# SADPR/1D-Burgers-Equation-ROMs

Hardware: AMD Instinct MI355X
Metric: batched Newton-steps/sec over mu-sweep (sample-Newton-steps/s, FOM N=1024) (higher is better)
Workload: dtype f64

## Files before the change

### 1d-burgers-equation-roms_amd/csrc/fom.hip

```cpp
#include <hip/hip_runtime.h>
#include <stdint.h>
#include <type_traits>

#include "../../include/burgers_hip.h"
#include "abi_common.hpp"
#include "fom_device.hpp"
#include "fom_wide.hpp"

namespace bg {
thread_local int tls_last_hip_error = 0;
}

namespace {

using namespace bg;

struct FomArgs {
    const double* x;
    const double* u0;
    const double* mu1;
    const double* mu2;
    double* hist;
    int32_t* iters;
    int32_t* flags;
    double dt, E, tol2;
    int N, B, nsteps, max_it, supg;
    double* errs;
};

constexpr int WAVES_PER_WG = 4;

template <int R>
__device__ __forceinline__ void load_rows(const double* __restrict__ src, int N, int row0, bool full,
                                          double (&u)[R])
{
#pragma unroll
    for (int j = 0; j < R; ++j) u[j] = (full || row0 + j < N) ? src[row0 + j] : 0.0;
}

template <int R>
__device__ __forceinline__ void store_rows(double* __restrict__ dst, int N, int row0, bool full,
                                           const double (&u)[R])
{
#pragma unroll
    for (int j = 0; j < R; ++j)
        if (full || row0 + j < N) dst[row0 + j] = u[j];
}

template <int R, bool FULL, bool UNI = true, bool TRACE = false>
__global__ __launch_bounds__(64 * WAVES_PER_WG, 1) void fom_fused_kernel(FomArgs a)
{
    const int lane = lane_id();
    const int s = blockIdx.x * WAVES_PER_WG + (int)(threadIdx.x >> 6);
    if (s >= a.B) return;
    const int N = a.N;
    const int row0 = lane * R;
    const double h = (a.x[N - 1] - a.x[0]) / (double)(N - 1);
    const MeshConst c = make_mesh_const(h, a.dt, a.E, a.supg);
    const double mu1 = a.mu1[s], mu2 = a.mu2[s];

    double hfs[R], fdt[R], u[R], g[R];
    ElemGeom<UNI ? 0 : R> gm;
    if constexpr (UNI) {
        forcing_setup<R>(a.x, N, row0, mu2, c.h, a.dt, hfs, fdt);
    } else {
        geom_setup<R>(a.x, N, row0, a.dt, a.E, gm);
        forcing_setup_general<R>(a.x, N, row0, mu2, a.dt, hfs, fdt);
    }

    double* hist = a.hist + (size_t)s * (size_t)(a.nsteps + 1) * (size_t)N;
    load_rows<R>(a.u0 + (size_t)s * N, N, row0, FULL, u);
    store_rows<R>(hist, N, row0, FULL, u);

    int flags = 0;
    for (int step = 0; step < a.nsteps; ++step) {
        if constexpr (UNI) mass_rhs<R, FULL>(c, N, row0, u, fdt, g);
        else mass_rhs_general<R>(gm, N, row0, u, fdt, g);
        int k = 0;
        bool more;
        do {
            double lo[R], di[R], up[R], rhs[R];
            if constexpr (UNI) assemble<R, FULL>(c, N, row0, mu1, u, g, hfs, lo, di, up, rhs);
            else assemble_general<R>(gm, a.dt, c.kap, N, row0, mu1, u, g, hfs, lo, di, up, rhs);
            tridiag_solve<R>(lo, di, up, rhs);
            double nd = 0.0, nu = 0.0;
#pragma unroll
            for (int j = 0; j < R; ++j) {
                u[j] += rhs[j];
                nd = __builtin_fma(rhs[j], rhs[j], nd);
                nu = __builtin_fma(u[j], u[j], nu);
            }
            wave_sum2(nd, nu, nd, nu);
            if constexpr (TRACE) {
                if (lane == 0) a.errs[((size_t)s * a.nsteps + step) * a.max_it + k] = sqrt(nd) / sqrt(nu);
            }
            ++k;
            more = (nd > a.tol2 * nu) && (k < a.max_it);
            if (!(nd - nd == 0.0) || !(nu - nu == 0.0)) flags |= BG_FLAG_NONFINITE;
        } while (more);
        if (k >= a.max_it) flags |= BG_FLAG_HIT_CAP;
        store_rows<R>(hist + (size_t)(step + 1) * N, N, row0, FULL, u);
        if (lane == 0) a.iters[(size_t)s * a.nsteps + step] = k;
    }
    if (lane == 0) a.flags[s] = flags;
}

struct AsmArgs {
    const double *x, *uk, *un, *mu1, *mu2;
    double *lo, *di, *up, *rhs;
    double dt, E;
    int N, B, supg;
};

template <int R, bool FULL, bool UNI = true>
__global__ __launch_bounds__(64 * WAVES_PER_WG, 1) void fom_assemble_kernel(AsmArgs a)
{
    const int lane = lane_id();
    const int s = blockIdx.x * WAVES_PER_WG + (int)(threadIdx.x >> 6);
    if (s >= a.B) return;
    const int N = a.N, row0 = lane * R;
    const double h = (a.x[N - 1] - a.x[0]) / (double)(N - 1);
    const MeshConst c = make_mesh_const(h, a.dt, a.E, a.supg);
    double hfs[R], fdt[R], u[R], un[R], g[R], lo[R], di[R], up[R], rhs[R];
    load_rows<R>(a.un + (size_t)s * N, N, row0, FULL, un);
    load_rows<R>(a.uk + (size_t)s * N, N, row0, FULL, u);
    if constexpr (UNI) {
        forcing_setup<R>(a.x, N, row0, a.mu2[s], c.h, a.dt, hfs, fdt);
        mass_rhs<R, FULL>(c, N, row0, un, fdt, g);
        assemble<R, FULL>(c, N, row0, a.mu1[s], u, g, hfs, lo, di, up, rhs);
    } else {
        ElemGeom<R> gm;
        geom_setup<R>(a.x, N, row0, a.dt, a.E, gm);
        forcing_setup_general<R>(a.x, N, row0, a.mu2[s], a.dt, hfs, fdt);
        mass_rhs_general<R>(gm, N, row0, un, fdt, g);
        assemble_general<R>(gm, a.dt, c.kap, N, row0, a.mu1[s], u, g, hfs, lo, di, up, rhs);
    }
    store_rows<R>(a.lo + (size_t)s * N, N, row0, FULL, lo);
    store_rows<R>(a.di + (size_t)s * N, N, row0, FULL, di);
    store_rows<R>(a.up + (size_t)s * N, N, row0, FULL, up);
    store_rows<R>(a.rhs + (size_t)s * N, N, row0, FULL, rhs);
}

struct SolveArgs {
    const double *lo, *di, *up, *rhs;
    double* sol;
    int N, B;
};

template <int R>
__global__ __launch_bounds__(64 * WAVES_PER_WG, 1) void tridiag_solve_kernel(SolveArgs a)
{
    const int lane = lane_id();
    const int s = blockIdx.x * WAVES_PER_WG + (int)(threadIdx.x >> 6);
    if (s >= a.B) return;
    const int N = a.N, row0 = lane * R;
    double lo[R], di[R], up[R], rhs[R];
    const size_t off = (size_t)s * N;
#pragma unroll
    for (int j = 0; j < R; ++j) {
        const bool in = row0 + j < N;
        lo[j] = in ? a.lo[off + row0 + j] : 0.0;
        di[j] = in ? a.di[off + row0 + j] : 1.0;
        up[j] = in ? a.up[off + row0 + j] : 0.0;
        rhs[j] = in ? a.rhs[off + row0 + j] : 0.0;
    }
    tridiag_solve<R>(lo, di, up, rhs);
    store_rows<R>(a.sol + off, N, row0, false, rhs);
}

template <int R, bool UNI>
__global__ __launch_bounds__(WIDE_THREADS, 1) void fom_wide_kernel(FomArgs a)
{
    constexpr bool PARK = UNI && R >= 32;
    __shared__ WideLds lds;
    __shared__ WidePark<PARK ? R : 1> park;
    const int g = threadIdx.x, s = blockIdx.x;
    const int N = a.N, row0 = g * R;
    wide_init(lds, g);
    const double h = (a.x[N - 1] - a.x[0]) / (double)(N - 1);
    const MeshConst c = make_mesh_const(h, a.dt, a.E, a.supg);
    const double mu1 = a.mu1[s], mu2 = a.mu2[s];
    double hfs[PARK ? 1 : R], fdt[R], u[R], gv[PARK ? 1 : R];
    ElemGeom<UNI ? 0 : R> gm;
    if constexpr (PARK) {
        double hf[R];
        forcing_setup<R>(a.x, N, row0, mu2, c.h, a.dt, hf, fdt);
#pragma unroll
        for (int j = 0; j < R; ++j) park.hfs[j][g] = hf[j];
    } else if constexpr (UNI) {
        forcing_setup<R>(a.x, N, row0, mu2, c.h, a.dt, hfs, fdt);
    } else {
        geom_setup<R>(a.x, N, row0, a.dt, a.E, gm);
        forcing_setup_general<R>(a.x, N, row0, mu2, a.dt, hfs, fdt);
    }
    double* hist = a.hist + (size_t)s * (size_t)(a.nsteps + 1) * (size_t)N;
    load_rows<R>(a.u0 + (size_t)s * N, N, row0, false, u);
    store_rows<R>(hist, N, row0, false, u);
    int flags = 0;
    for (int step = 0; step < a.nsteps; ++step) {
        if constexpr (PARK) wide_mass_rhs_uni_parked<R>(lds, park, g, c, N, u, fdt);
        else if constexpr (UNI) wide_mass_rhs_uni<R>(lds, g, c, N, u, fdt, gv);
        else wide_mass_rhs<R>(lds, g, gm, N, u, fdt, gv);
        int k = 0;
        bool more;
        do {
            double lo[R], di[R], up[R], rhs[R];
            if constexpr (PARK) wide_assemble_uni_parked<R>(lds, park, g, c, N, mu1, u, lo, di, up, rhs);
            else if constexpr (UNI) wide_assemble_uni<R>(lds, g, c, N, mu1, u, gv, hfs, lo, di, up, rhs);
            else wide_assemble<R>(lds, g, gm, a.dt, c.kap, N, mu1, u, gv, hfs, lo, di, up, rhs);
            wide_tridiag_solve<R>(lds, g, lo, di, up, rhs);
            double nd = 0.0, nu = 0.0;
#pragma unroll
            for (int j = 0; j < R; ++j) {
                u[j] += rhs[j];
                nd = __builtin_fma(rhs[j], rhs[j], nd);
                nu = __builtin_fma(u[j], u[j], nu);
            }
            wide_sum2(lds, g, nd, nu, nd, nu);
            ++k;
            more = (nd > a.tol2 * nu) && (k < a.max_it);
            if (!(nd - nd == 0.0) || !(nu - nu == 0.0)) flags |= BG_FLAG_NONFINITE;
        } while (more);
        if (k >= a.max_it) flags |= BG_FLAG_HIT_CAP;
        store_rows<R>(hist + (size_t)(step + 1) * N, N, row0, false, u);
        if (g == 0) a.iters[(size_t)s * a.nsteps + step] = k;
    }
    if (g == 0) a.flags[s] = flags;
}

template <int R, bool UNI>
__global__ __launch_bounds__(WIDE_THREADS, 1) void fom_assemble_wide_kernel(AsmArgs a)
{
    __shared__ WideLds lds;
    const int g = threadIdx.x, s = blockIdx.x;
    const int N = a.N, row0 = g * R;
    wide_init(lds, g);
    const double h = (a.x[N - 1] - a.x[0]) / (double)(N - 1);
    const MeshConst c = make_mesh_const(h, a.dt, a.E, a.supg);
    double hfs[R], fdt[R], u[R], un[R], gv[R], lo[R], di[R], up[R], rhs[R];
    load_rows<R>(a.un + (size_t)s * N, N, row0, false, un);
    load_rows<R>(a.uk + (size_t)s * N, N, row0, false, u);
    if constexpr (UNI) {
        forcing_setup<R>(a.x, N, row0, a.mu2[s], c.h, a.dt, hfs, fdt);
        wide_mass_rhs_uni<R>(lds, g, c, N, un, fdt, gv);
        wide_assemble_uni<R>(lds, g, c, N, a.mu1[s], u, gv, hfs, lo, di, up, rhs);
    } else {
        ElemGeom<R> gm;
        geom_setup<R>(a.x, N, row0, a.dt, a.E, gm);
        forcing_setup_general<R>(a.x, N, row0, a.mu2[s], a.dt, hfs, fdt);
        wide_mass_rhs<R>(lds, g, gm, N, un, fdt, gv);
        wide_assemble<R>(lds, g, gm, a.dt, c.kap, N, a.mu1[s], u, gv, hfs, lo, di, up, rhs);
    }
    store_rows<R>(a.lo + (size_t)s * N, N, row0, false, lo);
    store_rows<R>(a.di + (size_t)s * N, N, row0, false, di);
    store_rows<R>(a.up + (size_t)s * N, N, row0, false, up);
    store_rows<R>(a.rhs + (size_t)s * N, N, row0, false, rhs);
}

template <int R>
__global__ __launch_bounds__(WIDE_THREADS, 1) void tridiag_solve_wide_kernel(SolveArgs a)
{
    __shared__ WideLds lds;
    const int g = threadIdx.x, s = blockIdx.x;
    const int N = a.N, row0 = g * R;
    wide_init(lds, g);
    double lo[R], di[R], up[R], rhs[R];
    const size_t off = (size_t)s * N;
#pragma unroll
    for (int j = 0; j < R; ++j) {
        const bool in = row0 + j < N;
        lo[j] = in ? a.lo[off + row0 + j] : 0.0;
        di[j] = in ? a.di[off + row0 + j] : 1.0;
        up[j] = in ? a.up[off + row0 + j] : 0.0;
        rhs[j] = in ? a.rhs[off + row0 + j] : 0.0;
    }
    wide_tridiag_solve<R>(lds, g, lo, di, up, rhs);
    store_rows<R>(a.sol + off, N, row0, false, rhs);
}

__global__ __launch_bounds__(256) void transpose_kernel(const double* __restrict__ in,
                                                        double* __restrict__ out, int nb, int rows, int cols)
{
    __shared__ double tile[32][33];
    const int c0 = blockIdx.x * 32, r0 = blockIdx.y * 32;
    const int tx = threadIdx.x & 31, ty = threadIdx.x >> 5;
    for (int b = blockIdx.z; b < nb; b += gridDim.z) {
        const size_t base = (size_t)b * rows * cols;
#pragma unroll
        for (int k = 0; k < 32; k += 8) {
            int r = r0 + ty + k, cc = c0 + tx;
            if (r < rows && cc < cols) tile[ty + k][tx] = in[base + (size_t)r * cols + cc];
        }
        __syncthreads();
#pragma unroll
        for (int k = 0; k < 32; k += 8) {
            int cc = c0 + ty + k, r = r0 + tx;
            if (r < rows && cc < cols) out[base + (size_t)cc * rows + r] = tile[tx][ty + k];
        }
        __syncthreads();
    }
}

constexpr int kRowsPerLane[] = {1, 2, 3, 4, 5, 6, 8, 9, 10, 12, 16, 24};

int rows_per_lane(int N)
{
    for (int r : kRowsPerLane)
        if (N <= 64 * r) return r;
    return 0;
}

constexpr int kWaveMaxN = 64 * 24, kWideMaxN = WIDE_THREADS * 32;

template <typename F>
int dispatch_wide(int N, F&& f)
{
    if (N <= WIDE_THREADS * 2) return f(std::integral_constant<int, 2>{});
    if (N <= WIDE_THREADS * 4) return f(std::integral_constant<int, 4>{});
    if (N <= WIDE_THREADS * 8) return f(std::integral_constant<int, 8>{});
    if (N <= WIDE_THREADS * 12) return f(std::integral_constant<int, 12>{});
    if (N <= WIDE_THREADS * 16) return f(std::integral_constant<int, 16>{});
    if (N <= WIDE_THREADS * 24) return f(std::integral_constant<int, 24>{});
    if (N <= WIDE_THREADS * 32) return f(std::integral_constant<int, 32>{});
    return BG_ERR_UNSUPPORTED_N;
}

template <typename F>
int dispatch_r(int N, F&& f)
{
    switch (rows_per_lane(N)) {
        case 1: return f(std::integral_constant<int, 1>{});
        case 2: return f(std::integral_constant<int, 2>{});
        case 3: return f(std::integral_constant<int, 3>{});
        case 4: return f(std::integral_constant<int, 4>{});
        case 5: return f(std::integral_constant<int, 5>{});
        case 6: return f(std::integral_constant<int, 6>{});
        case 8: return f(std::integral_constant<int, 8>{});
        case 9: return f(std::integral_constant<int, 9>{});
        case 10: return f(std::integral_constant<int, 10>{});
        case 12: return f(std::integral_constant<int, 12>{});
        case 16: return f(std::integral_constant<int, 16>{});
        case 24: return f(std::integral_constant<int, 24>{});
        default: return BG_ERR_UNSUPPORTED_N;
    }
}

}

extern "C" {

int bg_abi_version(void) { return BG_ABI_VERSION; }

int bg_last_hip_error(void) { return bg::tls_last_hip_error; }

int bg_fom_max_n(void) { return kWideMaxN; }

const char* bg_strerror(int code)
{
    switch (code) {
        case BG_OK: return "ok";
        case BG_ERR_BAD_ARG: return "bad argument";
        case BG_ERR_UNSUPPORTED_N: return "N not supported by the fused kernels (2 <= N <= 8192)";
        case BG_ERR_NONUNIFORM: return "mesh is not uniform";
        case BG_ERR_LAUNCH: return "kernel launch failed (see bg_last_hip_error)";
        case BG_ERR_UNSUPPORTED_R: return "reduced dimension not supported";
        case BG_ERR_PROJECTION: return "unknown projection";
        case BG_ERR_WORKSPACE: return "workspace too small";
        default: return "unknown error";
    }
}

int bg_fom_run(int N, int B, int nsteps, const double* x, const double* u0, const double* mu1,
               const double* mu2, double dt, double E, double tol, int max_it, int supg, double* hist,
               int32_t* iters, int32_t* flags, void* stream)
{
    if (N < 2 || B < 0 || nsteps < 0 || max_it < 1 || !(dt > 0.0)) return BG_ERR_BAD_ARG;
    if (B == 0) return BG_OK;
    if (!x || !u0 || !mu1 || !mu2 || !hist || !flags || (nsteps > 0 && !iters)) return BG_ERR_BAD_ARG;
    FomArgs a;
    a.x = x; a.u0 = u0; a.mu1 = mu1; a.mu2 = mu2; a.hist = hist; a.iters = iters; a.flags = flags; a.errs = nullptr;
    a.dt = dt; a.E = E; a.tol2 = tol * tol;
    a.N = N; a.B = B; a.nsteps = nsteps; a.max_it = max_it; a.supg = supg & BG_OPT_SUPG;
    const bool nonuniform = (supg & BG_OPT_NONUNIFORM) != 0;
    const dim3 grid((B + WAVES_PER_WG - 1) / WAVES_PER_WG), block(64 * WAVES_PER_WG);
    hipStream_t st = (hipStream_t)stream;
    const bool both = N <= kWaveMaxN && N > 64 && !nonuniform;
    const bool wide = N > kWaveMaxN || (both && (supg & BG_OPT_FOM_WIDE) && !(supg & BG_OPT_FOM_WAVE));
    if (wide)
        return dispatch_wide(N, [&](auto rc) {
            constexpr int R = decltype(rc)::value;
            if constexpr (R >= 8) {
                if (nonuniform) {
                    hipLaunchKernelGGL((fom_wide_kernel<R, false>), dim3(B), dim3(WIDE_THREADS), 0, st, a);
                    return check_launch();
                }
            }
            hipLaunchKernelGGL((fom_wide_kernel<R, true>), dim3(B), dim3(WIDE_THREADS), 0, st, a);
            return check_launch();
        });
    return dispatch_r(N, [&](auto rc) {
        constexpr int R = decltype(rc)::value;
        if (nonuniform)
            hipLaunchKernelGGL((fom_fused_kernel<R, false, false>), grid, block, 0, st, a);
        else if (N == 64 * R)
            hipLaunchKernelGGL((fom_fused_kernel<R, true>), grid, block, 0, st, a);
        else
            hipLaunchKernelGGL((fom_fused_kernel<R, false>), grid, block, 0, st, a);
        return check_launch();
    });
}

int bg_fom_run_traced(int N, int B, int nsteps, const double* x, const double* u0, const double* mu1, const double* mu2,
                      double dt, double E, double tol, int max_it, int supg, double* hist, int32_t* iters, int32_t* flags,
                      double* errs, void* stream)
{
    if (N < 2 || B < 0 || nsteps < 0 || max_it < 1 || !(dt > 0.0)) return BG_ERR_BAD_ARG;
    if (N > kWaveMaxN) return BG_ERR_UNSUPPORTED_N;
    if (B == 0) return BG_OK;
    if (!x || !u0 || !mu1 || !mu2 || !hist || !flags || !errs || (nsteps > 0 && !iters)) return BG_ERR_BAD_ARG;
    FomArgs a;
    a.x = x; a.u0 = u0; a.mu1 = mu1; a.mu2 = mu2; a.hist = hist; a.iters = iters; a.flags = flags; a.errs = errs;
    a.dt = dt; a.E = E; a.tol2 = tol * tol;
    a.N = N; a.B = B; a.nsteps = nsteps; a.max_it = max_it; a.supg = supg & BG_OPT_SUPG;
    const bool nonuniform = (supg & BG_OPT_NONUNIFORM) != 0;
    const dim3 grid((B + WAVES_PER_WG - 1) / WAVES_PER_WG), block(64 * WAVES_PER_WG);
    hipStream_t st = (hipStream_t)stream;
    return dispatch_r(N, [&](auto rc) {
        constexpr int R = decltype(rc)::value;
        if (nonuniform)
            hipLaunchKernelGGL((fom_fused_kernel<R, false, false, true>), grid, block, 0, st, a);
        else
            hipLaunchKernelGGL((fom_fused_kernel<R, false, true, true>), grid, block, 0, st, a);
        return check_launch();
    });
}

int bg_fom_assemble(int N, int B, const double* x, const double* uk, const double* un, const double* mu1,
                    const double* mu2, double dt, double E, int supg, double* lo, double* di, double* up,
                    double* rhs, void* stream)
{
    if (N < 2 || B < 0 || !(dt > 0.0)) return BG_ERR_BAD_ARG;
    if (B == 0) return BG_OK;
    if (!x || !uk || !un || !mu1 || !mu2 || !lo || !di || !up || !rhs) return BG_ERR_BAD_ARG;
    AsmArgs a;
    a.x = x; a.uk = uk; a.un = un; a.mu1 = mu1; a.mu2 = mu2; a.lo = lo; a.di = di; a.up = up; a.rhs = rhs;
    a.dt = dt; a.E = E; a.N = N; a.B = B; a.supg = supg & BG_OPT_SUPG;
    const bool nonuniform = (supg & BG_OPT_NONUNIFORM) != 0;
    const dim3 grid((B + WAVES_PER_WG - 1) / WAVES_PER_WG), block(64 * WAVES_PER_WG);
    hipStream_t st = (hipStream_t)stream;
    if (N > kWaveMaxN)
        return dispatch_wide(N, [&](auto rc) {
            constexpr int R = decltype(rc)::value;
            if (nonuniform)
                hipLaunchKernelGGL((fom_assemble_wide_kernel<R, false>), dim3(B), dim3(WIDE_THREADS), 0, st, a);
            else
                hipLaunchKernelGGL((fom_assemble_wide_kernel<R, true>), dim3(B), dim3(WIDE_THREADS), 0, st, a);
            return check_launch();
        });
    return dispatch_r(N, [&](auto rc) {
        constexpr int R = decltype(rc)::value;
        if (nonuniform)
            hipLaunchKernelGGL((fom_assemble_kernel<R, false, false>), grid, block, 0, st, a);
        else if (N == 64 * R)
            hipLaunchKernelGGL((fom_assemble_kernel<R, true>), grid, block, 0, st, a);
        else
            hipLaunchKernelGGL((fom_assemble_kernel<R, false>), grid, block, 0, st, a);
        return check_launch();
    });
}

int bg_tridiag_solve(int N, int B, const double* lo, const double* di, const double* up, const double* rhs,
                     double* sol, void* stream)
{
    if (N < 1 || B < 0) return BG_ERR_BAD_ARG;
    if (B == 0) return BG_OK;
    if (!lo || !di || !up || !rhs || !sol) return BG_ERR_BAD_ARG;
    SolveArgs a{lo, di, up, rhs, sol, N, B};
    const dim3 grid((B + WAVES_PER_WG - 1) / WAVES_PER_WG), block(64 * WAVES_PER_WG);
    hipStream_t st = (hipStream_t)stream;
    if (N > kWaveMaxN)
        return dispatch_wide(N, [&](auto rc) {
            constexpr int R = decltype(rc)::value;
            hipLaunchKernelGGL((tridiag_solve_wide_kernel<R>), dim3(B), dim3(WIDE_THREADS), 0, st, a);
            return check_launch();
        });
    return dispatch_r(N, [&](auto rc) {
        constexpr int R = decltype(rc)::value;
        hipLaunchKernelGGL((tridiag_solve_kernel<R>), grid, block, 0, st, a);
        return check_launch();
    });
}

int bg_transpose_batched(int B, int rows, int cols, const double* in, double* out, void* stream)
{
    if (B < 0 || rows < 0 || cols < 0) return BG_ERR_BAD_ARG;
    if (B == 0 || rows == 0 || cols == 0) return BG_OK;
    if (!in || !out) return BG_ERR_BAD_ARG;
    const dim3 grid((cols + 31) / 32, (rows + 31) / 32, B < 65535 ? B : 65535), block(256);
    hipLaunchKernelGGL(transpose_kernel, grid, block, 0, (hipStream_t)stream, in, out, B, rows, cols);
    return check_launch();
}

}
```

### 1d-burgers-equation-roms_amd/csrc/fom_device.hpp

```cpp
#pragma once
#include "wave_ops.hpp"

#ifndef BG_RCP
#define BG_RCP rcp1
#endif

namespace bg {

constexpr double GP_A = 0.78867513459481287;
constexpr double GP_B = 0.21132486540518713;

struct MeshConst {
    double h;
    double aoff;
    double dd2;
    double dd1;
    double dt6;
    double kap;
    double h6;
};

__device__ __forceinline__ MeshConst make_mesh_const(double h, double dt, double E, int supg)
{
    MeshConst c;
    c.h = h;
    double eh = dt * E / h;
    c.aoff = h / 6.0 - eh;
    c.dd1 = h / 3.0 + eh;
    c.dd2 = 2.0 * c.dd1;
    c.dt6 = dt / 6.0;
    c.kap = supg ? 0.25 * dt : 0.0;
    c.h6 = h / 6.0;
    return c;
}

template <int R>
__device__ __forceinline__ void forcing_setup(const double* __restrict__ x, int N, int row0, double mu2,
                                              double h, double dt, double (&hfs)[R], double (&fdt)[R])
{
    double frPrev = 0.0;
    {
        int e = row0 - 1;
        if (e >= 0 && e < N - 1) {
            double xl = x[e], xr = x[e + 1];
            double f1 = 0.02 * exp(mu2 * (GP_A * xl + GP_B * xr));
            double f2 = 0.02 * exp(mu2 * (GP_B * xl + GP_A * xr));
            frPrev = (f1 * GP_B + f2 * GP_A) * (0.5 * h);
        }
    }
#pragma unroll
    for (int j = 0; j < R; ++j) {
        int e = row0 + j;
        double fl = 0.0, fr = 0.0, fs = 0.0;
        if (e < N - 1) {
            double xl = x[e], xr = x[e + 1];
            double f1 = 0.02 * exp(mu2 * (GP_A * xl + GP_B * xr));
            double f2 = 0.02 * exp(mu2 * (GP_B * xl + GP_A * xr));
            fl = (f1 * GP_A + f2 * GP_B) * (0.5 * h);
            fr = (f1 * GP_B + f2 * GP_A) * (0.5 * h);
            fs = f1 + f2;
        }
        hfs[j] = h * fs;
        fdt[j] = (e < N) ? dt * (frPrev + fl) : 0.0;
        frPrev = fr;
    }
}

template <int R, bool FULL, typename GStore>
__device__ __forceinline__ void mass_rhs_core_to(const MeshConst& c, int N, int row0, const double (&u)[R], double uL,
                                                 double uR, const double (&fdt)[R], GStore&& gstore)
{
#pragma unroll
    for (int j = 0; j < R; ++j) {
        const double um = (j == 0) ? uL : u[j - 1];
        const double up = (j == R - 1) ? uR : u[j + 1];
        const int i = row0 + j;
        double inner = __builtin_fma(4.0, u[j], um) + up;
        double last = __builtin_fma(2.0, u[j], um);
        double v = __builtin_fma(c.h6, (i == N - 1) ? last : inner, fdt[j]);
        gstore(j, (!FULL && i >= N) ? 0.0 : v);
    }
}

template <int R, bool FULL>
__device__ __forceinline__ void mass_rhs_core(const MeshConst& c, int N, int row0, const double (&u)[R], double uL,
                                              double uR, const double (&fdt)[R], double (&g)[R])
{
    mass_rhs_core_to<R, FULL>(c, N, row0, u, uL, uR, fdt, [&](int j, double v) { g[j] = v; });
}

template <int R, bool FULL>
__device__ __forceinline__ void mass_rhs(const MeshConst& c, int N, int row0, const double (&u)[R],
                                         const double (&fdt)[R], double (&g)[R])
{
    mass_rhs_core<R, FULL>(c, N, row0, u, from_lane_below(u[R - 1]), from_lane_above(u[0]), fdt, g);
}

template <int R, typename HF>
__device__ __forceinline__ void assemble_p1_from(const MeshConst& c, const double (&u)[R], double uL, double uR,
                                                 HF&& hf, double (&lo)[R], double (&up)[R], double (&se)[R])
{
#pragma unroll
    for (int j = 0; j < R; ++j) {
        const double ur = (j == R - 1) ? uR : u[j + 1];
        const double w = u[j] + ur;
        const double dif = ur - u[j];
        up[j] = __builtin_fma(c.dt6, w + u[j], c.aoff);
        if (j + 1 < R) lo[j + 1] = __builtin_fma(-c.dt6, w + ur, c.aoff);
        const double mx = fmax(fabs(w), 2.0e-10);
        const double t = __builtin_fma(w, dif, -hf(j));
        se[j] = t * BG_RCP(mx);
    }
    lo[0] = __builtin_fma(-c.dt6, __builtin_fma(2.0, u[0], uL), c.aoff);
}

template <int R>
__device__ __forceinline__ void assemble_p1(const MeshConst& c, const double (&u)[R], double uL, double uR,
                                            const double (&hfs)[R], double (&lo)[R], double (&up)[R],
                                            double (&se)[R])
{
    assemble_p1_from<R>(c, u, uL, uR, [&](int j) { return hfs[j]; }, lo, up, se);
}

template <int R, bool FULL, typename GF>
__device__ __forceinline__ void assemble_p2_from(const MeshConst& c, int N, int row0, bool first, bool last_lane,
                                                 double mu1, const double (&u)[R], double uL, double uR, double seL,
                                                 GF&& g, const double (&se)[R], double (&lo)[R],
                                                 double (&di)[R], double (&up)[R], double (&rhs)[R])
{
#pragma unroll
    for (int j = 0; j < R; ++j) {
        const double um = (j == 0) ? uL : u[j - 1];
        const double ur = (j == R - 1) ? uR : u[j + 1];
        const double sm = (j == 0) ? seL : se[j - 1];
        const int i = row0 + j;
        double d = __builtin_fma(c.dt6, um - ur, c.dd2);
        double b = __builtin_fma(-c.kap, sm, g(j));
        double bb = __builtin_fma(c.kap, se[j], b);
        double l = lo[j], p = up[j];
        const bool is_last = FULL ? (j == R - 1 && last_lane) : (i == N - 1);
        if (FULL ? (j == R - 1) : true) {
            double dl = __builtin_fma(c.dt6, __builtin_fma(2.0, u[j], um), c.dd1);
            d = is_last ? dl : d;
            p = is_last ? 0.0 : p;
            bb = is_last ? b : bb;
        }
        if (!FULL) {
            const bool pad = i >= N;
            d = pad ? 1.0 : d;
            p = pad ? 0.0 : p;
            l = pad ? 0.0 : l;
            bb = pad ? 0.0 : bb;
        }
        if (j == 0) {
            d = first ? 1.0 : d;
            p = first ? 0.0 : p;
            l = first ? 0.0 : l;
            bb = first ? mu1 : bb;
        }
        double r = __builtin_fma(-l, um, bb);
        r = __builtin_fma(-d, u[j], r);
        r = __builtin_fma(-p, ur, r);
        lo[j] = l; di[j] = d; up[j] = p; rhs[j] = r;
    }
}

template <int R, bool FULL>
__device__ __forceinline__ void assemble_p2(const MeshConst& c, int N, int row0, bool first, bool last_lane,
                                            double mu1, const double (&u)[R], double uL, double uR, double seL,
                                            const double (&g)[R], const double (&se)[R], double (&lo)[R],
                                            double (&di)[R], double (&up)[R], double (&rhs)[R])
{
    assemble_p2_from<R, FULL>(c, N, row0, first, last_lane, mu1, u, uL, uR, seL, [&](int j) { return g[j]; }, se, lo, di,
                              up, rhs);
}

template <int R, bool FULL>
__device__ __forceinline__ void assemble(const MeshConst& c, int N, int row0, double mu1,
                                         const double (&u)[R], const double (&g)[R],
                                         const double (&hfs)[R], double (&lo)[R], double (&di)[R],
                                         double (&up)[R], double (&rhs)[R])
{
    const int lane = lane_id();
    const double uL = from_lane_below(u[R - 1]);
    const double uR = from_lane_above(u[0]);
    double se[R];
    assemble_p1<R>(c, u, uL, uR, hfs, lo, up, se);
    const double seL = from_lane_below(se[R - 1]);
    assemble_p2<R, FULL>(c, N, row0, lane == 0, lane == 63, mu1, u, uL, uR, seL, g, se, lo, di, up, rhs);
}

template <int R>
struct ElemGeom {
    double h6[R + 1];
    double eh[R + 1];
};

template <int R>
__device__ __forceinline__ void geom_setup(const double* __restrict__ x, int N, int row0, double dt, double E,
                                           ElemGeom<R>& gm)
{
#pragma unroll
    for (int j = 0; j <= R; ++j) {
        const int e = row0 + j - 1;
        double h = 1.0;
        if (e >= 0 && e < N - 1) h = x[e + 1] - x[e];
        gm.h6[j] = (e >= 0 && e < N - 1) ? h / 6.0 : 0.0;
        gm.eh[j] = (e >= 0 && e < N - 1) ? dt * E / h : 0.0;
    }
}

template <int R>
__device__ __forceinline__ void forcing_setup_general(const double* __restrict__ x, int N, int row0, double mu2,
                                                      double dt, double (&hfs)[R], double (&fdt)[R])
{
    double frPrev = 0.0;
#pragma unroll
    for (int j = -1; j < R; ++j) {
        const int e = row0 + j;
        double fl = 0.0, fr = 0.0, hf = 0.0;
        if (e >= 0 && e < N - 1) {
            const double xl = x[e], xr = x[e + 1], h = xr - xl;
            const double f1 = 0.02 * exp(mu2 * (GP_A * xl + GP_B * xr));
            const double f2 = 0.02 * exp(mu2 * (GP_B * xl + GP_A * xr));
            fl = (f1 * GP_A + f2 * GP_B) * (0.5 * h);
            fr = (f1 * GP_B + f2 * GP_A) * (0.5 * h);
            hf = h * (f1 + f2);
        }
        if (j >= 0) {
            hfs[j] = hf;
            fdt[j] = (e < N) ? dt * (frPrev + fl) : 0.0;
        }
        frPrev = fr;
    }
}

template <int R>
__device__ __forceinline__ void mass_rhs_general_core(const ElemGeom<R>& gm, int N, int row0, const double (&u)[R],
                                                      double uL, double uR, const double (&fdt)[R], double (&g)[R])
{
#pragma unroll
    for (int j = 0; j < R; ++j) {
        const double um = (j == 0) ? uL : u[j - 1];
        const double up = (j == R - 1) ? uR : u[j + 1];
        const int i = row0 + j;
        double v = gm.h6[j] * __builtin_fma(2.0, u[j], um);
        v = __builtin_fma(gm.h6[j + 1], __builtin_fma(2.0, u[j], up), v);
        g[j] = (i >= N) ? 0.0 : v + fdt[j];
    }
}

template <int R>
__device__ __forceinline__ void mass_rhs_general(const ElemGeom<R>& gm, int N, int row0, const double (&u)[R],
                                                 const double (&fdt)[R], double (&g)[R])
{
    mass_rhs_general_core<R>(gm, N, row0, u, from_lane_below(u[R - 1]), from_lane_above(u[0]), fdt, g);
}

template <int R>
__device__ __forceinline__ void assemble_general_p1(const ElemGeom<R>& gm, double dt, const double (&u)[R], double uL,
                                                    double uR, const double (&hfs)[R], double (&lo)[R],
                                                    double (&up)[R], double (&se)[R])
{
    const double dt6 = dt / 6.0;
#pragma unroll
    for (int j = 0; j < R; ++j) {
        const double ur = (j == R - 1) ? uR : u[j + 1];
        const double w = u[j] + ur;
        const double dif = ur - u[j];
        const double aoff = gm.h6[j + 1] - gm.eh[j + 1];
        up[j] = __builtin_fma(dt6, w + u[j], aoff);
        if (j + 1 < R) lo[j + 1] = __builtin_fma(-dt6, w + ur, aoff);
        const double mx = fmax(fabs(w), 2.0e-10);
        const double t = __builtin_fma(w, dif, -hfs[j]);
        se[j] = t * BG_RCP(mx);
    }
    lo[0] = __builtin_fma(-dt6, __builtin_fma(2.0, u[0], uL), gm.h6[0] - gm.eh[0]);
}

template <int R>
__device__ __forceinline__ void assemble_general_p2(const ElemGeom<R>& gm, double dt, double kap, int N, int row0,
                                                    bool first, double mu1, const double (&u)[R], double uL,
                                                    double uR, double seL, const double (&g)[R],
                                                    const double (&se)[R], double (&lo)[R], double (&di)[R],
                                                    double (&up)[R], double (&rhs)[R])
{
    const double dt6 = dt / 6.0;
#pragma unroll
    for (int j = 0; j < R; ++j) {
        const double um = (j == 0) ? uL : u[j - 1];
        const double ur = (j == R - 1) ? uR : u[j + 1];
        const double sm = (j == 0) ? seL : se[j - 1];
        const int i = row0 + j;
        const double ddl = __builtin_fma(2.0, gm.h6[j], gm.eh[j]);
        const double ddr = __builtin_fma(2.0, gm.h6[j + 1], gm.eh[j + 1]);
        double d = __builtin_fma(dt6, um - ur, ddl + ddr);
        double b = __builtin_fma(-kap, sm, g[j]);
        double bb = __builtin_fma(kap, se[j], b);
        double l = lo[j], p = up[j];
        const bool is_last = (i == N - 1);
        const double dl = __builtin_fma(dt6, __builtin_fma(2.0, u[j], um), ddl);
        d = is_last ? dl : d;
        p = is_last ? 0.0 : p;
        bb = is_last ? b : bb;
        const bool pad = i >= N;
        d = pad ? 1.0 : d;
        p = pad ? 0.0 : p;
        l = pad ? 0.0 : l;
        bb = pad ? 0.0 : bb;
        if (j == 0) {
            d = first ? 1.0 : d;
            p = first ? 0.0 : p;
            l = first ? 0.0 : l;
            bb = first ? mu1 : bb;
        }
        double r = __builtin_fma(-l, um, bb);
        r = __builtin_fma(-d, u[j], r);
        r = __builtin_fma(-p, ur, r);
        lo[j] = l; di[j] = d; up[j] = p; rhs[j] = r;
    }
}

template <int R>
__device__ __forceinline__ void assemble_general(const ElemGeom<R>& gm, double dt, double kap, int N, int row0,
                                                 double mu1, const double (&u)[R], const double (&g)[R],
                                                 const double (&hfs)[R], double (&lo)[R], double (&di)[R],
                                                 double (&up)[R], double (&rhs)[R])
{
    const double uL = from_lane_below(u[R - 1]);
    const double uR = from_lane_above(u[0]);
    double se[R];
    assemble_general_p1<R>(gm, dt, u, uL, uR, hfs, lo, up, se);
    const double seL = from_lane_below(se[R - 1]);
    assemble_general_p2<R>(gm, dt, kap, N, row0, lane_id() == 0, mu1, u, uL, uR, seL, g, se, lo, di, up, rhs);
}

template <int CTRL_DN, int CTRL_UP, int REPS, bool LAST>
__device__ __forceinline__ void pcr_step(double& A, double& C, double& D)
{
    const double Dm = dpp_shift<CTRL_DN, REPS>(D), Dp = dpp_shift<CTRL_UP, REPS>(D);
    const double Cm = dpp_shift<CTRL_DN, REPS>(C), Ap = dpp_shift<CTRL_UP, REPS>(A);
    double Bn = __builtin_fma(-Cm, A, 1.0);
    Bn = __builtin_fma(-Ap, C, Bn);
    double Dn = __builtin_fma(-Dm, A, D);
    Dn = __builtin_fma(-Dp, C, Dn);
    const double rb = BG_RCP(Bn);
    D = Dn * rb;
    if (!LAST) {
        const double Am = dpp_shift<CTRL_DN, REPS>(A), Cp = dpp_shift<CTRL_UP, REPS>(C);
        A = -(Am * A) * rb;
        C = -(Cp * C) * rb;
    }
}

template <int R>
__device__ __forceinline__ double wang_reduce(double (&lo)[R], double (&di)[R], const double (&up)[R],
                                              double (&rhs)[R], double (&gs)[R])
{
    static_assert(R > 1, "R == 1 has no interior rows");
    double dp = di[0];
    di[0] = BG_RCP(dp);
#pragma unroll
    for (int j = 1; j < R; ++j) {
        const double m = lo[j] * di[j - 1];
        dp = __builtin_fma(-m, up[j - 1], di[j]);
        di[j] = BG_RCP(dp);
        rhs[j] = __builtin_fma(-m, rhs[j - 1], rhs[j]);
        lo[j] = -m * lo[j - 1];
    }
    gs[R - 2] = up[R - 2];
#pragma unroll
    for (int j = R - 3; j >= 0; --j) {
        const double t = up[j] * di[j + 1];
        rhs[j] = __builtin_fma(-t, rhs[j + 1], rhs[j]);
        lo[j] = __builtin_fma(-t, lo[j + 1], lo[j]);
        gs[j] = -t * gs[j + 1];
    }
    return dp;
}

template <int R>
__device__ __forceinline__ void wang_interface(const double (&lo)[R], const double (&up)[R], const double (&rhs)[R],
                                               double dp, double F0, double G0, double R0, double& A, double& C,
                                               double& D)
{
    const double ul = up[R - 1];
    const double B = __builtin_fma(-ul, F0, dp);
    const double rb = BG_RCP(B);
    A = lo[R - 1] * rb;
    C = -(ul * G0) * rb;
    D = __builtin_fma(-ul, R0, rhs[R - 1]) * rb;
}

template <int R>
__device__ __forceinline__ void wang_finish(const double (&lo)[R], const double (&di)[R], double (&rhs)[R],
                                            const double (&gs)[R], double X, double XL)
{
#pragma unroll
    for (int j = 0; j < R - 1; ++j) {
        double v = __builtin_fma(-lo[j], XL, rhs[j]);
        v = __builtin_fma(-gs[j], X, v);
        rhs[j] = v * di[j];
    }
    rhs[R - 1] = X;
}

__device__ __forceinline__ double pcr64(double A, double C, double D)
{
    const int lane = lane_id();
    pcr_step<0x138, 0x130, 1, false>(A, C, D);
    pcr_step<0x138, 0x130, 2, false>(A, C, D);
    {
        const int src = ((4 * (lane & 15) + (lane >> 4)) << 2);
        A = from_lane_rot(A, src); C = from_lane_rot(C, src); D = from_lane_rot(D, src);
    }
    pcr_step<0x111, 0x101, 1, false>(A, C, D);
    pcr_step<0x112, 0x102, 1, false>(A, C, D);
    pcr_step<0x114, 0x104, 1, false>(A, C, D);
    pcr_step<0x118, 0x108, 1, true>(A, C, D);
    return from_lane_rot(D, (16 * (lane & 3) + (lane >> 2)) << 2);
}

template <int R>
__device__ __forceinline__ void tridiag_solve(double (&lo)[R], double (&di)[R], const double (&up)[R],
                                              double (&rhs)[R])
{
    if constexpr (R == 1) {
        const double rb = BG_RCP(di[0]);
        rhs[0] = pcr64(lo[0] * rb, up[0] * rb, rhs[0] * rb);
    } else {
        double gs[R];
        const double dp = wang_reduce<R>(lo, di, up, rhs, gs);
        const double F0 = from_lane_above(lo[0] * di[0]);
        const double G0 = from_lane_above(gs[0] * di[0]);
        const double R0 = from_lane_above(rhs[0] * di[0]);
        double A, C, D;
        wang_interface<R>(lo, up, rhs, dp, F0, G0, R0, A, C, D);
        const double X = pcr64(A, C, D);
        wang_finish<R>(lo, di, rhs, gs, X, from_lane_below(X));
    }
}

}
```

### 1d-burgers-equation-roms_amd/csrc/fom_wide.hpp

```cpp
#pragma once
#include "fom_device.hpp"

namespace bg {

constexpr int WIDE_WAVES = 4;
constexpr int WIDE_THREADS = 64 * WIDE_WAVES;
constexpr int WIDE_PAD = 2;
constexpr int WIDE_LEN = WIDE_THREADS + 2 * WIDE_PAD;

struct WideLds {
    double ufirst[WIDE_LEN], ulast[WIDE_LEN];
    double se[WIDE_LEN];
    double fgr[3][WIDE_LEN];
    double pcr[2][3][WIDE_LEN];
    double x[WIDE_LEN];
    double nrm[2][WIDE_WAVES];
};

__device__ __forceinline__ void wide_init(WideLds& s, int tid)
{
    double* p = reinterpret_cast<double*>(&s);
    for (int i = tid; i < (int)(sizeof(WideLds) / sizeof(double)); i += WIDE_THREADS) p[i] = 0.0;
    __syncthreads();
}

template <int R>
__device__ __forceinline__ void wide_halo_u(WideLds& s, int g, const double (&u)[R], double& uL, double& uR)
{
    s.ufirst[g + WIDE_PAD] = u[0];
    s.ulast[g + WIDE_PAD] = u[R - 1];
    __syncthreads();
    uL = s.ulast[g + WIDE_PAD - 1];
    uR = s.ufirst[g + WIDE_PAD + 1];
}

template <int R>
__device__ __forceinline__ void wide_mass_rhs(WideLds& s, int g, const ElemGeom<R>& gm, int N, const double (&u)[R],
                                              const double (&fdt)[R], double (&gv)[R])
{
    double uL, uR;
    wide_halo_u<R>(s, g, u, uL, uR);
    mass_rhs_general_core<R>(gm, N, g * R, u, uL, uR, fdt, gv);
    __syncthreads();
}

template <int R>
__device__ __forceinline__ void wide_assemble(WideLds& s, int g, const ElemGeom<R>& gm, double dt, double kap, int N,
                                              double mu1, const double (&u)[R], const double (&gv)[R],
                                              const double (&hfs)[R], double (&lo)[R], double (&di)[R],
                                              double (&up)[R], double (&rhs)[R])
{
    double uL, uR, se[R];
    wide_halo_u<R>(s, g, u, uL, uR);
    assemble_general_p1<R>(gm, dt, u, uL, uR, hfs, lo, up, se);
    s.se[g + WIDE_PAD] = se[R - 1];
    __syncthreads();
    const double seL = s.se[g + WIDE_PAD - 1];
    assemble_general_p2<R>(gm, dt, kap, N, g * R, g == 0, mu1, u, uL, uR, seL, gv, se, lo, di, up, rhs);
}

template <int R>
struct WidePark {
    double g[R][WIDE_THREADS];
    double hfs[R][WIDE_THREADS];
};

template <int R>
__device__ __forceinline__ void wide_mass_rhs_uni_parked(WideLds& s, WidePark<R>& pk, int g, const MeshConst& c, int N,
                                                         const double (&u)[R], const double (&fdt)[R])
{
    double uL, uR;
    wide_halo_u<R>(s, g, u, uL, uR);
    mass_rhs_core_to<R, false>(c, N, g * R, u, uL, uR, fdt, [&](int j, double v) { pk.g[j][g] = v; });
    __syncthreads();
}

template <int R>
__device__ __forceinline__ void wide_assemble_uni_parked(WideLds& s, const WidePark<R>& pk, int g, const MeshConst& c, int N,
                                                         double mu1, const double (&u)[R], double (&lo)[R], double (&di)[R],
                                                         double (&up)[R], double (&rhs)[R])
{
    double uL, uR, se[R];
    wide_halo_u<R>(s, g, u, uL, uR);
    assemble_p1_from<R>(c, u, uL, uR, [&](int j) { return pk.hfs[j][g]; }, lo, up, se);
    s.se[g + WIDE_PAD] = se[R - 1];
    __syncthreads();
    const double seL = s.se[g + WIDE_PAD - 1];
    assemble_p2_from<R, false>(c, N, g * R, g == 0, false, mu1, u, uL, uR, seL, [&](int j) { return pk.g[j][g]; }, se, lo,
                               di, up, rhs);
}

template <int R>
__device__ __forceinline__ void wide_mass_rhs_uni(WideLds& s, int g, const MeshConst& c, int N, const double (&u)[R],
                                                  const double (&fdt)[R], double (&gv)[R])
{
    double uL, uR;
    wide_halo_u<R>(s, g, u, uL, uR);
    mass_rhs_core<R, false>(c, N, g * R, u, uL, uR, fdt, gv);
    __syncthreads();
}

template <int R>
__device__ __forceinline__ void wide_assemble_uni(WideLds& s, int g, const MeshConst& c, int N, double mu1,
                                                  const double (&u)[R], const double (&gv)[R],
                                                  const double (&hfs)[R], double (&lo)[R], double (&di)[R],
                                                  double (&up)[R], double (&rhs)[R])
{
    double uL, uR, se[R];
    wide_halo_u<R>(s, g, u, uL, uR);
    assemble_p1<R>(c, u, uL, uR, hfs, lo, up, se);
    s.se[g + WIDE_PAD] = se[R - 1];
    __syncthreads();
    const double seL = s.se[g + WIDE_PAD - 1];
    assemble_p2<R, false>(c, N, g * R, g == 0, false, mu1, u, uL, uR, seL, gv, se, lo, di, up, rhs);
}

template <int S>
__device__ __forceinline__ void wide_pcr_step(const double (&buf)[3][WIDE_LEN], int e, double& A, double& C, double& D)
{
    const int m = e + WIDE_PAD - S, p = e + WIDE_PAD + S;
    const double Am = buf[0][m], Cm = buf[1][m], Dm = buf[2][m];
    const double Ap = buf[0][p], Cp = buf[1][p], Dp = buf[2][p];
    double Bn = __builtin_fma(-Cm, A, 1.0);
    Bn = __builtin_fma(-Ap, C, Bn);
    double Dn = __builtin_fma(-Dm, A, D);
    Dn = __builtin_fma(-Dp, C, Dn);
    const double rb = BG_RCP(Bn);
    D = Dn * rb;
    A = -(Am * A) * rb;
    C = -(Cp * C) * rb;
}

template <int R>
__device__ __forceinline__ void wide_tridiag_solve(WideLds& s, int g, double (&lo)[R], double (&di)[R],
                                                   const double (&up)[R], double (&rhs)[R])
{
    double gs[R];
    const double dp = wang_reduce<R>(lo, di, up, rhs, gs);
    s.fgr[0][g + WIDE_PAD] = lo[0] * di[0];
    s.fgr[1][g + WIDE_PAD] = gs[0] * di[0];
    s.fgr[2][g + WIDE_PAD] = rhs[0] * di[0];
    __syncthreads();
    double A, C, D;
    wang_interface<R>(lo, up, rhs, dp, s.fgr[0][g + WIDE_PAD + 1], s.fgr[1][g + WIDE_PAD + 1],
                      s.fgr[2][g + WIDE_PAD + 1], A, C, D);
    s.pcr[0][0][g + WIDE_PAD] = A;
    s.pcr[0][1][g + WIDE_PAD] = C;
    s.pcr[0][2][g + WIDE_PAD] = D;
    __syncthreads();
    const int e = (g & 63) * WIDE_WAVES + (g >> 6);
    A = s.pcr[0][0][e + WIDE_PAD]; C = s.pcr[0][1][e + WIDE_PAD]; D = s.pcr[0][2][e + WIDE_PAD];
    wide_pcr_step<1>(s.pcr[0], e, A, C, D);
    s.pcr[1][0][e + WIDE_PAD] = A;
    s.pcr[1][1][e + WIDE_PAD] = C;
    s.pcr[1][2][e + WIDE_PAD] = D;
    __syncthreads();
    wide_pcr_step<2>(s.pcr[1], e, A, C, D);
    s.x[e + WIDE_PAD] = pcr64(A, C, D);
    __syncthreads();
    wang_finish<R>(lo, di, rhs, gs, s.x[g + WIDE_PAD], s.x[g + WIDE_PAD - 1]);
}

__device__ __forceinline__ void wide_sum2(WideLds& s, int g, double a, double b, double& sa, double& sb)
{
    wave_sum2(a, b, a, b);
    if ((g & 63) == 0) { s.nrm[0][g >> 6] = a; s.nrm[1][g >> 6] = b; }
    __syncthreads();
    sa = (s.nrm[0][0] + s.nrm[0][1]) + (s.nrm[0][2] + s.nrm[0][3]);
    sb = (s.nrm[1][0] + s.nrm[1][1]) + (s.nrm[1][2] + s.nrm[1][3]);
}

}
```

### 1d-burgers-equation-roms_amd/csrc/wave_ops.hpp

```cpp
#pragma once
#include <hip/hip_runtime.h>

namespace bg {

constexpr int WAVE = 64;

__device__ __forceinline__ int lane_id() { return (int)(threadIdx.x & 63u); }

template <int CTRL, int ROW_MASK = 0xF, bool BOUND_ZERO = true>
__device__ __forceinline__ double dpp_mov(double v, double old = 0.0)
{
    int lo = __double2loint(v), hi = __double2hiint(v);
    int olo = __double2loint(old), ohi = __double2hiint(old);
    lo = __builtin_amdgcn_update_dpp(olo, lo, CTRL, ROW_MASK, 0xF, BOUND_ZERO);
    hi = __builtin_amdgcn_update_dpp(ohi, hi, CTRL, ROW_MASK, 0xF, BOUND_ZERO);
    return __hiloint2double(hi, lo);
}

__device__ __forceinline__ double from_lane_below(double v) { return dpp_mov<0x138>(v); }
__device__ __forceinline__ double from_lane_above(double v) { return dpp_mov<0x130>(v); }

__device__ __forceinline__ double from_lane_rot(double v, int src_lane_times4)
{
    int lo = __double2loint(v), hi = __double2hiint(v);
    lo = __builtin_amdgcn_ds_bpermute(src_lane_times4, lo);
    hi = __builtin_amdgcn_ds_bpermute(src_lane_times4, hi);
    return __hiloint2double(hi, lo);
}

__device__ __forceinline__ double wave_sum(double v)
{
    v += dpp_mov<0x111>(v);
    v += dpp_mov<0x112>(v);
    v += dpp_mov<0x114>(v);
    v += dpp_mov<0x118>(v);
    v += dpp_mov<0x142, 0xA>(v);
    v += dpp_mov<0x143, 0xC>(v);
    int lo = __builtin_amdgcn_readlane(__double2loint(v), 63);
    int hi = __builtin_amdgcn_readlane(__double2hiint(v), 63);
    return __hiloint2double(hi, lo);
}

__device__ __forceinline__ double rcp(double d)
{
    double r = __builtin_amdgcn_rcp(d);
    double e = __builtin_fma(-d, r, 1.0);
    r = __builtin_fma(r, e, r);
    e = __builtin_fma(-d, r, 1.0);
    r = __builtin_fma(r, e, r);
    return r;
}

__device__ __forceinline__ double rcp1(double d)
{
    double r = __builtin_amdgcn_rcp(d);
    double e = __builtin_fma(-d, r, 1.0);
    return __builtin_fma(r, e, r);
}

template <int CTRL, int REPS>
__device__ __forceinline__ double dpp_shift(double v)
{
#pragma unroll
    for (int i = 0; i < REPS; ++i) v = dpp_mov<CTRL>(v);
    return v;
}

__device__ __forceinline__ void wave_sum2(double a, double b, double& sa, double& sb)
{
    auto l = __builtin_amdgcn_permlane32_swap((unsigned)__double2loint(a), (unsigned)__double2loint(b), false, false);
    auto h = __builtin_amdgcn_permlane32_swap((unsigned)__double2hiint(a), (unsigned)__double2hiint(b), false, false);
    double v = __hiloint2double((int)h[0], (int)l[0]) + __hiloint2double((int)h[1], (int)l[1]);
    v += dpp_mov<0x111>(v);
    v += dpp_mov<0x112>(v);
    v += dpp_mov<0x114>(v);
    v += dpp_mov<0x118>(v);
    v += dpp_mov<0x142, 0xA>(v);
    sa = __hiloint2double(__builtin_amdgcn_readlane(__double2hiint(v), 31),
                          __builtin_amdgcn_readlane(__double2loint(v), 31));
    sb = __hiloint2double(__builtin_amdgcn_readlane(__double2hiint(v), 63),
                          __builtin_amdgcn_readlane(__double2loint(v), 63));
}

__device__ __forceinline__ double sel(bool c, double a, double b) { return c ? a : b; }

}
```

Baseline: 572.8 million.

## Batch SUPG reciprocals via product-tree inversion and hoist phase-1 assembly

```diff
diff --git a/1d-burgers-equation-roms_amd/csrc/fom.hip b/1d-burgers-equation-roms_amd/csrc/fom.hip
--- a/1d-burgers-equation-roms_amd/csrc/fom.hip
+++ b/1d-burgers-equation-roms_amd/csrc/fom.hip
@@ -72,16 +72,29 @@
     load_rows<R>(a.u0 + (size_t)s * N, N, row0, FULL, u);
     store_rows<R>(hist, N, row0, FULL, u);
 
+    double lo[R], up[R], se[R];
+    double uL = from_lane_below(u[R - 1]), uR = from_lane_above(u[0]);
+    bool p1_ok;
+    if constexpr (UNI) p1_ok = assemble_p1<R>(c, u, uL, uR, hfs, lo, up, se);
+    else p1_ok = assemble_general_p1<R>(gm, a.dt, u, uL, uR, hfs, lo, up, se);
+
     int flags = 0;
     for (int step = 0; step < a.nsteps; ++step) {
-        if constexpr (UNI) mass_rhs<R, FULL>(c, N, row0, u, fdt, g);
-        else mass_rhs_general<R>(gm, N, row0, u, fdt, g);
+        if constexpr (UNI) mass_rhs_core<R, FULL>(c, N, row0, u, uL, uR, fdt, g);
+        else mass_rhs_general_core<R>(gm, N, row0, u, uL, uR, fdt, g);
         int k = 0;
         bool more;
         do {
-            double lo[R], di[R], up[R], rhs[R];
-            if constexpr (UNI) assemble<R, FULL>(c, N, row0, mu1, u, g, hfs, lo, di, up, rhs);
-            else assemble_general<R>(gm, a.dt, c.kap, N, row0, mu1, u, g, hfs, lo, di, up, rhs);
+            if (!p1_ok) {
+                if constexpr (UNI) assemble_p1<R, 1>(c, u, uL, uR, hfs, lo, up, se);
+                else assemble_general_p1<R, 1>(gm, a.dt, u, uL, uR, hfs, lo, up, se);
+            }
+            double di[R], rhs[R];
+            const double seL = from_lane_below(se[R - 1]);
+            if constexpr (UNI)
+                assemble_p2<R, FULL>(c, N, row0, lane == 0, lane == 63, mu1, u, uL, uR, seL, g, se, lo, di, up, rhs);
+            else
+                assemble_general_p2<R>(gm, a.dt, c.kap, N, row0, lane == 0, mu1, u, uL, uR, seL, g, se, lo, di, up, rhs);
             tridiag_solve<R>(lo, di, up, rhs);
             double nd = 0.0, nu = 0.0;
 #pragma unroll
@@ -90,6 +103,10 @@
                 nd = __builtin_fma(rhs[j], rhs[j], nd);
                 nu = __builtin_fma(u[j], u[j], nu);
             }
+            uL = from_lane_below(u[R - 1]);
+            uR = from_lane_above(u[0]);
+            if constexpr (UNI) p1_ok = assemble_p1<R>(c, u, uL, uR, hfs, lo, up, se);
+            else p1_ok = assemble_general_p1<R>(gm, a.dt, u, uL, uR, hfs, lo, up, se);
             wave_sum2(nd, nu, nd, nu);
             if constexpr (TRACE) {
                 if (lane == 0) a.errs[((size_t)s * a.nsteps + step) * a.max_it + k] = sqrt(nd) / sqrt(nu);
diff --git a/1d-burgers-equation-roms_amd/csrc/fom_device.hpp b/1d-burgers-equation-roms_amd/csrc/fom_device.hpp
--- a/1d-burgers-equation-roms_amd/csrc/fom_device.hpp
+++ b/1d-burgers-equation-roms_amd/csrc/fom_device.hpp
@@ -96,10 +96,20 @@
     mass_rhs_core<R, FULL>(c, N, row0, u, from_lane_below(u[R - 1]), from_lane_above(u[0]), fdt, g);
 }
 
-template <int R, typename HF>
-__device__ __forceinline__ void assemble_p1_from(const MeshConst& c, const double (&u)[R], double uL, double uR,
+#ifndef BG_SE_GROUP
+#define BG_SE_GROUP 4
+#endif
+template <int G, int R>
+__device__ __forceinline__ bool se_quotients(const double (&mx)[R], const double (&t)[R], double (&se)[R])
+{
+    return quot_batch<G, R>(mx, t, se, [](double d) { return BG_RCP(d); });
+}
+
+template <int R, int G = BG_SE_GROUP, typename HF>
+__device__ __forceinline__ bool assemble_p1_from(const MeshConst& c, const double (&u)[R], double uL, double uR,
                                                  HF&& hf, double (&lo)[R], double (&up)[R], double (&se)[R])
 {
+    double mx[R], t[R];
 #pragma unroll
     for (int j = 0; j < R; ++j) {
         const double ur = (j == R - 1) ? uR : u[j + 1];
@@ -107,19 +117,20 @@
         const double dif = ur - u[j];
         up[j] = __builtin_fma(c.dt6, w + u[j], c.aoff);
         if (j + 1 < R) lo[j + 1] = __builtin_fma(-c.dt6, w + ur, c.aoff);
-        const double mx = fmax(fabs(w), 2.0e-10);
-        const double t = __builtin_fma(w, dif, -hf(j));
-        se[j] = t * BG_RCP(mx);
-    }
+        mx[j] = fmax(fabs(w), 2.0e-10);
+        t[j] = __builtin_fma(w, dif, -hf(j));
+    }
+    const bool ok = se_quotients<G, R>(mx, t, se);
     lo[0] = __builtin_fma(-c.dt6, __builtin_fma(2.0, u[0], uL), c.aoff);
-}
-
-template <int R>
-__device__ __forceinline__ void assemble_p1(const MeshConst& c, const double (&u)[R], double uL, double uR,
+    return ok;
+}
+
+template <int R, int G = BG_SE_GROUP>
+__device__ __forceinline__ bool assemble_p1(const MeshConst& c, const double (&u)[R], double uL, double uR,
                                             const double (&hfs)[R], double (&lo)[R], double (&up)[R],
                                             double (&se)[R])
 {
-    assemble_p1_from<R>(c, u, uL, uR, [&](int j) { return hfs[j]; }, lo, up, se);
+    return assemble_p1_from<R, G>(c, u, uL, uR, [&](int j) { return hfs[j]; }, lo, up, se);
 }
 
 template <int R, bool FULL, typename GF>
@@ -185,7 +196,7 @@
     const double uL = from_lane_below(u[R - 1]);
     const double uR = from_lane_above(u[0]);
     double se[R];
-    assemble_p1<R>(c, u, uL, uR, hfs, lo, up, se);
+    if (!assemble_p1<R>(c, u, uL, uR, hfs, lo, up, se)) assemble_p1<R, 1>(c, u, uL, uR, hfs, lo, up, se);
     const double seL = from_lane_below(se[R - 1]);
     assemble_p2<R, FULL>(c, N, row0, lane == 0, lane == 63, mu1, u, uL, uR, seL, g, se, lo, di, up, rhs);
 }
@@ -257,12 +268,13 @@
     mass_rhs_general_core<R>(gm, N, row0, u, from_lane_below(u[R - 1]), from_lane_above(u[0]), fdt, g);
 }
 
-template <int R>
-__device__ __forceinline__ void assemble_general_p1(const ElemGeom<R>& gm, double dt, const double (&u)[R], double uL,
+template <int R, int G = BG_SE_GROUP>
+__device__ __forceinline__ bool assemble_general_p1(const ElemGeom<R>& gm, double dt, const double (&u)[R], double uL,
                                                     double uR, const double (&hfs)[R], double (&lo)[R],
                                                     double (&up)[R], double (&se)[R])
 {
     const double dt6 = dt / 6.0;
+    double mx[R], t[R];
 #pragma unroll
     for (int j = 0; j < R; ++j) {
         const double ur = (j == R - 1) ? uR : u[j + 1];
@@ -271,11 +283,12 @@
         const double aoff = gm.h6[j + 1] - gm.eh[j + 1];
         up[j] = __builtin_fma(dt6, w + u[j], aoff);
         if (j + 1 < R) lo[j + 1] = __builtin_fma(-dt6, w + ur, aoff);
-        const double mx = fmax(fabs(w), 2.0e-10);
-        const double t = __builtin_fma(w, dif, -hfs[j]);
-        se[j] = t * BG_RCP(mx);
-    }
+        mx[j] = fmax(fabs(w), 2.0e-10);
+        t[j] = __builtin_fma(w, dif, -hfs[j]);
+    }
+    const bool ok = se_quotients<G, R>(mx, t, se);
     lo[0] = __builtin_fma(-dt6, __builtin_fma(2.0, u[0], uL), gm.h6[0] - gm.eh[0]);
+    return ok;
 }
 
 template <int R>
@@ -330,7 +343,7 @@
     const double uL = from_lane_below(u[R - 1]);
     const double uR = from_lane_above(u[0]);
     double se[R];
-    assemble_general_p1<R>(gm, dt, u, uL, uR, hfs, lo, up, se);
+    if (!assemble_general_p1<R>(gm, dt, u, uL, uR, hfs, lo, up, se)) assemble_general_p1<R, 1>(gm, dt, u, uL, uR, hfs, lo, up, se);
     const double seL = from_lane_below(se[R - 1]);
     assemble_general_p2<R>(gm, dt, kap, N, row0, lane_id() == 0, mu1, u, uL, uR, seL, g, se, lo, di, up, rhs);
 }
diff --git a/1d-burgers-equation-roms_amd/csrc/fom_wide.hpp b/1d-burgers-equation-roms_amd/csrc/fom_wide.hpp
--- a/1d-burgers-equation-roms_amd/csrc/fom_wide.hpp
+++ b/1d-burgers-equation-roms_amd/csrc/fom_wide.hpp
@@ -52,7 +52,8 @@
 {
     double uL, uR, se[R];
     wide_halo_u<R>(s, g, u, uL, uR);
-    assemble_general_p1<R>(gm, dt, u, uL, uR, hfs, lo, up, se);
+    if (!assemble_general_p1<R>(gm, dt, u, uL, uR, hfs, lo, up, se))
+        assemble_general_p1<R, 1>(gm, dt, u, uL, uR, hfs, lo, up, se);
     s.se[g + WIDE_PAD] = se[R - 1];
     __syncthreads();
     const double seL = s.se[g + WIDE_PAD - 1];
@@ -82,7 +83,8 @@
 {
     double uL, uR, se[R];
     wide_halo_u<R>(s, g, u, uL, uR);
-    assemble_p1_from<R>(c, u, uL, uR, [&](int j) { return pk.hfs[j][g]; }, lo, up, se);
+    if (!assemble_p1_from<R>(c, u, uL, uR, [&](int j) { return pk.hfs[j][g]; }, lo, up, se))
+        assemble_p1_from<R, 1>(c, u, uL, uR, [&](int j) { return pk.hfs[j][g]; }, lo, up, se);
     s.se[g + WIDE_PAD] = se[R - 1];
     __syncthreads();
     const double seL = s.se[g + WIDE_PAD - 1];
@@ -108,7 +110,7 @@
 {
     double uL, uR, se[R];
     wide_halo_u<R>(s, g, u, uL, uR);
-    assemble_p1<R>(c, u, uL, uR, hfs, lo, up, se);
+    if (!assemble_p1<R>(c, u, uL, uR, hfs, lo, up, se)) assemble_p1<R, 1>(c, u, uL, uR, hfs, lo, up, se);
     s.se[g + WIDE_PAD] = se[R - 1];
     __syncthreads();
     const double seL = s.se[g + WIDE_PAD - 1];
diff --git a/1d-burgers-equation-roms_amd/csrc/wave_ops.hpp b/1d-burgers-equation-roms_amd/csrc/wave_ops.hpp
--- a/1d-burgers-equation-roms_amd/csrc/wave_ops.hpp
+++ b/1d-burgers-equation-roms_amd/csrc/wave_ops.hpp
@@ -58,6 +58,59 @@
     return __builtin_fma(r, e, r);
 }
 
+namespace detail {
+template <int O, int G, int R, typename Rcp>
+__device__ __forceinline__ void quot_group(const double (&d)[R], const double (&t)[R], double (&q)[R], Rcp& rcpf,
+                                           bool& ok)
+{
+    if constexpr (G == 1) {
+        q[O] = t[O] * rcpf(d[O]);
+    } else {
+        double p[2 * G];
+#pragma unroll
+        for (int j = 0; j < G; ++j) p[G + j] = d[O + j];
+#pragma unroll
+        for (int k = G - 1; k >= 1; --k) p[k] = p[2 * k] * p[2 * k + 1];
+        ok = ok & (p[1] < 0x1p1000);
+        double inv[G];
+        inv[1] = rcpf(p[1]);
+#pragma unroll
+        for (int k = 1; k < G / 2; ++k) {
+            inv[2 * k] = inv[k] * p[2 * k + 1];
+            inv[2 * k + 1] = inv[k] * p[2 * k];
+        }
+#pragma unroll
+        for (int j = 0; j < G; ++j) {
+            const int leaf = G + j;
+            q[O + j] = t[O + j] * (p[leaf ^ 1] * inv[leaf >> 1]);
+        }
+    }
+}
+
+template <int O, int G, int R, typename Rcp>
+__device__ __forceinline__ void quot_groups(const double (&d)[R], const double (&t)[R], double (&q)[R], Rcp& rcpf,
+                                            bool& ok)
+{
+    if constexpr (O < R) {
+        if constexpr (O + G <= R) {
+            quot_group<O, G, R>(d, t, q, rcpf, ok);
+            quot_groups<O + G, G, R>(d, t, q, rcpf, ok);
+        } else {
+            quot_groups<O, G / 2, R>(d, t, q, rcpf, ok);
+        }
+    }
+}
+}
+
+template <int G, int R, typename Rcp>
+__device__ __forceinline__ bool quot_batch(const double (&d)[R], const double (&t)[R], double (&q)[R], Rcp&& rcpf)
+{
+    static_assert(G >= 1 && (G & (G - 1)) == 0, "group size must be a power of two");
+    bool ok = true;
+    detail::quot_groups<0, G, R>(d, t, q, rcpf, ok);
+    return ok;
+}
+
 template <int CTRL, int REPS>
 __device__ __forceinline__ double dpp_shift(double v)
 {
```

New measurement: 573.4 million (median of 6 runs). About the same (+0.1%).
